# camillabelponer/dealii-slod

Measured on NVIDIA B200. Metric: slod_basis_patches_per_s, higher is better.
Workload: dtype f64

## Files before the change

### dealii-slod_b200/csrc/kernels.cu

```cuda
#include <cuda_runtime.h>
#include <math.h>
#include <stdint.h>
#include <stdio.h>
#include <stdlib.h>

#include "geom.h"
#include "kernels.h"

namespace slod {

__constant__ Params cP;

cudaError_t upload_params(const Params &p, cudaStream_t st) {
  return cudaMemcpyToSymbolAsync(cP, &p, sizeof(Params), 0, cudaMemcpyHostToDevice, st);
}

__device__ __forceinline__ int nfields() { return cP.problem == 0 ? 1 : 2; }

__device__ void load_coef(const Geom &g, const double *__restrict__ d_coef, double *sCoef, int t0 = -1, int nt = 0) {
  if (t0 < 0) { t0 = threadIdx.x; nt = blockDim.x; }
  const int n = cP.n;
  const int msx = g.m[0] * n, msy = g.m[1] * n, msz = (cP.dim == 3) ? g.m[2] * n : 1;
  const int nsubp = msx * msy * msz;
  const long long nsub = cP.nsub;
// ... 790 lines not shown
        x0[j] = max(gq.lo[0] * n, ulo[0]);
        x1[j] = min((gq.lo[0] + gq.m[0]) * n, uhi[0]);
        if (x1[j] < x0[j]) continue;
        qid[j] = (int)morton_fast(qc, DIM);
        lox[j] = gq.lo[0] * n;
        px[j] = gq.p[0];
        ux0 = min(ux0, x0[j]);
        ux1 = max(ux1, x1[j]);
        if (!got) {
          got = true;
          b0y = max(gq.lo[1] * n, ulo[1]);
          b1y = min((gq.lo[1] + gq.m[1]) * n, uhi[1]);
          loy = gq.lo[1] * n;
          py = gq.p[1];
          if (DIM == 3) {
            b0z = max(gq.lo[2] * n, ulo[2]);
            b1z = min((gq.lo[2] + gq.m[2]) * n, uhi[2]);
            loz = gq.lo[2] * n;
          } else {
            b0z = 0; b1z = 0; loz = 0;
          }
        }
      }
      if (!got || b1y < b0y || b1z < b0z) continue;
      const int exu = ux1 - ux0 + 1, ey = b1y - b0y + 1, ez = b1z - b0z + 1;
      for (int e = 0; e < S; ++e) {
        double acc[NQ][NA];
#pragma unroll
        for (int j = 0; j < NQ; ++j)
#pragma unroll
          for (int k = 0; k < NA; ++k) acc[j][k] = 0.0;
        for (int t = lane; t < exu * ey; t += 32) {
          const int iy = t / exu, ix = t - iy * exu;
          const int gx = ux0 + ix, gy = b0y + iy;
          const double *u1 = sU + (((b0z - ulo[2]) * NU + (gy - ulo[1])) * NU + (gx - ulo[0])) * S;
          const double *q1[NQ];
          int sq[NQ];
          bool in[NQ];
#pragma unroll
          for (int j = 0; j < NQ; ++j) {
            in[j] = gx >= x0[j] && gx <= x1[j];
            sq[j] = px[j] * py * S;
            q1[j] = aphi + ((size_t)qid[j] * S + e) * lay.nf_max +
                    (((b0z - loz) * py + (gy - loy)) * px[j] + (in[j] ? gx - lox[j] : 0)) * S;
          }
          for (int iz = 0; iz < ez; ++iz) {
#pragma unroll
            for (int c = 0; c < S; ++c) {
              double v[NQ];
#pragma unroll
              for (int j = 0; j < NQ; ++j) v[j] = in[j] ? q1[j][iz * sq[j] + c] : 0.0;
              const double *u = u1 + iz * NU * NU * S + c;
#pragma unroll
              for (int k = 0; k < NA; ++k) {
                const double uk = u[(size_t)k * NUV * S];
#pragma unroll
                for (int j = 0; j < NQ; ++j) acc[j][k] += v[j] * uk;
              }
            }
          }
        }
#pragma unroll
        for (int j = 0; j < NQ; ++j) {
          if (x1[j] < x0[j]) continue;
          const double val = warp_sum_packed(acc[j], lane);
          if ((lane & (NA == 8 ? 3 : 7)) == 0) {
            const int k = warp_sum_index<NA>(lane);
            const int mem = k / S, d = k - mem * S;
            if (sGeo[mem][7]) {
              const int Dx = qx0 + j - sGeo[mem][3], Dy = qy - sGeo[mem][4], Dz = (DIM == 3) ? qz - sGeo[mem][5] : 0;
              if (abs(Dx) <= w && abs(Dy) <= w && abs(Dz) <= w) {
                const int slot = (DIM == 3) ? ((Dz + w) * ww + (Dy + w)) * ww + (Dx + w) : (Dy + w) * ww + (Dx + w);
                Kell[((size_t)sGeo[mem][6] * S + d) * cP.ell_width + slot * S + e] = val;
              }
            }
          }
        }
      }
    }
  }
}
template <int DIM, int S>
static cudaError_t launch_coarse_blocked_t(int grid, size_t smem, cudaStream_t st, int p0, int p1, const double *phi,
                                           const double *aphi, double *Kell, const FinishLayout &lay, int NU,
                                           const int *groups, int n_groups) {
  if (groups) {
    cudaError_t e = cudaFuncSetAttribute(k_coarse_blocked<DIM, S, true>, cudaFuncAttributeMaxDynamicSharedMemorySize, (int)smem);
    if (e != cudaSuccess) return e;
    k_coarse_blocked<DIM, S, true><<<grid, kCoarseThreads, smem, st>>>(p0, p1, groups, n_groups, phi, aphi, Kell, lay, NU);
    return cudaGetLastError();
  }
  cudaError_t e = cudaFuncSetAttribute(k_coarse_blocked<DIM, S, false>, cudaFuncAttributeMaxDynamicSharedMemorySize, (int)smem);
  if (e != cudaSuccess) return e;
  e = cudaMemsetAsync(Kell + (size_t)p0 * S * (lay.ell_width), 0, sizeof(double) * (size_t)(p1 - p0) * S * lay.ell_width, st);
  if (e != cudaSuccess) return e;
  k_coarse_blocked<DIM, S, false><<<grid, kCoarseThreads, smem, st>>>(p0, p1, nullptr, 0, phi, aphi, Kell, lay, NU);
  return cudaGetLastError();
}
size_t coarse_blocked_smem(int dim, int s, int NU) {
  size_t nuv = (dim == 3) ? (size_t)NU * NU * NU : (size_t)NU * NU;
  return sizeof(double) * ((size_t)(1 << dim) * s * nuv * s);
}
cudaError_t launch_coarse_blocked(int dim, int s, int grid, size_t smem, cudaStream_t st, int p0, int p1,
                                  const double *phi, const double *aphi, double *Kell, const FinishLayout &lay, int NU,
                                  const int *groups, int n_groups) {
  if (dim == 3 && s == 1) return launch_coarse_blocked_t<3, 1>(grid, smem, st, p0, p1, phi, aphi, Kell, lay, NU, groups, n_groups);
  if (dim == 2 && s == 1) return launch_coarse_blocked_t<2, 1>(grid, smem, st, p0, p1, phi, aphi, Kell, lay, NU, groups, n_groups);
  if (dim == 2 && s == 2) return launch_coarse_blocked_t<2, 2>(grid, smem, st, p0, p1, phi, aphi, Kell, lay, NU, groups, n_groups);
  return cudaErrorInvalidValue;
}

cudaError_t launch_patch_solve(int grid, size_t smem, cudaStream_t st, const int *ids, int n_work, const double *coef,
                               double *X, double *Lws, int *status, const SolveLayout &lay) {
  cudaError_t e = cudaFuncSetAttribute(k_patch_solve<kSolveNB>, cudaFuncAttributeMaxDynamicSharedMemorySize, (int)smem);
  if (e != cudaSuccess) return e;
  k_patch_solve<kSolveNB><<<grid, lay.threads, smem, st>>>(ids, n_work, coef, X, Lws, status, lay);
  return cudaGetLastError();
}
template <int RBMAX, int NW>
static cudaError_t launch_mma_t(int grid, size_t smem, cudaStream_t st, const int *ids, int n_work, const double *coef,
                                double *X, double *Lws, int *status, const SolveMmaLayout &lay, int *work_counter) {
  cudaError_t e = cudaFuncSetAttribute(k_patch_solve_mma<RBMAX, NW>, cudaFuncAttributeMaxDynamicSharedMemorySize, (int)smem);
  if (e != cudaSuccess) return e;
  k_patch_solve_mma<RBMAX, NW><<<grid, 32 * NW, smem, st>>>(ids, n_work, coef, X, Lws, status, lay, work_counter);
  return cudaGetLastError();
}
size_t solve_mma_smem(int variant, int coef_doubles, int nip_max, int stw) {
  const int RBMAX = (variant == 0) ? 13 : 4;
  const int NW = (variant == 0) ? 16 : (variant == 1 ? 4 : 8);
  const int R = 8 * RBMAX, LDWF = (R % 16 == 8) ? R : R + 8, LDP = R + 4;
  return sizeof(double) * ((size_t)coef_doubles + (size_t)R * LDWF + 8 * LDP + kSolveStages * (R * 8 + 64) +
                           (size_t)nip_max * stw) +
         sizeof(int) * ((size_t)nip_max + 8 * NW + RBMAX * (RBMAX - 1) / 2 + 32 + 8);
}
cudaError_t launch_patch_solve_mma(int variant, int grid, size_t smem, cudaStream_t st, const int *ids, int n_work,
                                   const double *coef, double *X, double *Lws, int *status, int coef_doubles, int ldx,
                                   long long x_stride, long long lws_per_cta, int nip_max, int stw, int *work_counter) {
  SolveMmaLayout lay{coef_doubles, nip_max, stw, ldx, x_stride, lws_per_cta};
  if (work_counter) {
    cudaError_t e = cudaMemsetAsync(work_counter, 0, sizeof(int), st);
    if (e != cudaSuccess) return e;
  }
  switch (variant) {
    case 0: return launch_mma_t<13, 16>(grid, smem, st, ids, n_work, coef, X, Lws, status, lay, work_counter);
    case 1: return launch_mma_t<4, 4>(grid, smem, st, ids, n_work, coef, X, Lws, status, lay, work_counter);
    case 2: return launch_mma_t<4, 8>(grid, smem, st, ids, n_work, coef, X, Lws, status, lay, work_counter);
  }
  return cudaErrorInvalidValue;
}

constexpr int kSplitRB = 13, kFactorWarps = 8, kTriWarps = 16;
size_t split_factor_smem(int coef_doubles, int nip_max) {
  const int R = 8 * kSplitRB, LDWF = (R % 16 == 8) ? R : R + 8, LDP = R + 4;
  return sizeof(double) * ((size_t)coef_doubles + (size_t)R * LDWF + 8 * LDP + 2 * 64 + 64) +
         sizeof(int) * ((size_t)nip_max + kSplitRB * (kSplitRB - 1) / 2 + 16 + 8);
}
size_t split_trisolve_smem(int nip_max) {
  return sizeof(double) * ((size_t)kTriStages * kSplitRB * 64) + 2 * kTriStages * sizeof(unsigned long long) +
         sizeof(int) * ((size_t)nip_max + 8 * kTriWarps + kTriWarps + nip_max / 8 + 1 + 8 + 4);
}
long long split_rec_stride(int nip_max) { return (long long)(nip_max / 8) * kSplitRB * 64; }
size_t split_stencil_ws_doubles(int grid, int nip_max) { return (size_t)grid * nip_max * 14; }
cudaError_t launch_patch_factor(int grid, size_t smem, cudaStream_t st, const int *ids, int n_work, const double *coef,
                                double *Lrec, double *stencil_ws, int *status, int coef_doubles, int nip_max, int ldx,
                                long long x_stride, int *work_counter) {
  SplitLayout lay{coef_doubles, nip_max, ldx, x_stride, split_rec_stride(nip_max)};
  cudaError_t e = cudaFuncSetAttribute(k_patch_factor<kSplitRB, kFactorWarps>, cudaFuncAttributeMaxDynamicSharedMemorySize, (int)smem);
  if (e != cudaSuccess) return e;
  e = cudaFuncSetAttribute(k_patch_factor<kSplitRB, kFactorWarps>, cudaFuncAttributePreferredSharedMemoryCarveout,
                           (int)cudaSharedmemCarveoutMaxShared);
  if (e != cudaSuccess) return e;
  if (getenv("SLOD_PRINT_OCC")) {
    int nb = 0;
    cudaOccupancyMaxActiveBlocksPerMultiprocessor(&nb, k_patch_factor<kSplitRB, kFactorWarps>, 32 * kFactorWarps, smem);
    printf("k_patch_factor: %d CTAs/SM, %zu B dynamic shared memory\n", nb, smem);
  }
  if (work_counter && (e = cudaMemsetAsync(work_counter, 0, sizeof(int), st)) != cudaSuccess) return e;
  k_patch_factor<kSplitRB, kFactorWarps><<<grid, 32 * kFactorWarps, smem, st>>>(ids, n_work, coef, Lrec, stencil_ws, status, lay, work_counter);
  return cudaGetLastError();
}
cudaError_t launch_patch_trisolve(int grid, size_t smem, cudaStream_t st, const int *ids, int n_work, const double *Lrec,
                                  double *X, int coef_doubles, int nip_max, int ldx, long long x_stride, int *work_counter) {
  SplitLayout lay{coef_doubles, nip_max, ldx, x_stride, split_rec_stride(nip_max)};
  cudaError_t e = cudaFuncSetAttribute(k_patch_trisolve<kSplitRB, kTriWarps>, cudaFuncAttributeMaxDynamicSharedMemorySize, (int)smem);
  if (e != cudaSuccess) return e;
  if (work_counter && (e = cudaMemsetAsync(work_counter, 0, sizeof(int), st)) != cudaSuccess) return e;
  k_patch_trisolve<kSplitRB, kTriWarps><<<grid, 32 * kTriWarps, smem, st>>>(ids, n_work, Lrec, X, lay, work_counter);
  return cudaGetLastError();
}

cudaError_t launch_patch_dense(int grid, size_t smem, cudaStream_t st, const int *ids, int n_work, const double *coef,
                               const double *X, double *Minv, double *G, double *diag, int *status,
                               const DenseLayout &lay) {
  cudaError_t e = cudaFuncSetAttribute(k_patch_dense, cudaFuncAttributeMaxDynamicSharedMemorySize, (int)smem);
  if (e != cudaSuccess) return e;
  k_patch_dense<<<grid, lay.threads, smem, st>>>(ids, n_work, coef, X, Minv, G, diag, status, lay);
  return cudaGetLastError();
}
template <int NTILE>
static cudaError_t launch_dense_t(int grid, size_t smem, cudaStream_t st, const int *ids, int n_work, const double *coef,
                                  const double *X, const double *W, double *Minv, double *G, double *diag, int *status,
                                  const DenseLayout &lay, int *work_counter) {
  cudaError_t e = cudaFuncSetAttribute(k_patch_dense_mma<NTILE>, cudaFuncAttributeMaxDynamicSharedMemorySize, (int)smem);
  if (e != cudaSuccess) return e;
  k_patch_dense_mma<NTILE><<<grid, 32 * NTILE, smem, st>>>(ids, n_work, coef, X, W, Minv, G, diag, status, lay, work_counter);
  return cudaGetLastError();
}
size_t dense_mma_smem(int ntile, int coef_doubles, int nb_max) {
  (void)nb_max;
  (void)coef_doubles;
  const int NC = 8 * ntile, LDM = NC + 4;
  return sizeof(double) * ((size_t)NC * LDM + 2 * (size_t)kDTB * LDM) + sizeof(int) * ((size_t)NC * 32 + 8);
}
cudaError_t launch_patch_dense_mma(int ntile, int grid, size_t smem, cudaStream_t st, const int *ids, int n_work,
                                   const double *coef, const double *X, const double *W, double *Minv, double *G,
                                   double *diag, int *status, const DenseLayout &lay, int *work_counter) {
  if (work_counter) {
    cudaError_t e = cudaMemsetAsync(work_counter, 0, sizeof(int), st);
    if (e != cudaSuccess) return e;
  }
  switch (ntile) {
    case 4: return launch_dense_t<4>(grid, smem, st, ids, n_work, coef, X, W, Minv, G, diag, status, lay, work_counter);
    case 8: return launch_dense_t<8>(grid, smem, st, ids, n_work, coef, X, W, Minv, G, diag, status, lay, work_counter);
    case 16: return launch_dense_t<16>(grid, smem, st, ids, n_work, coef, X, W, Minv, G, diag, status, lay, work_counter);
  }
  return cudaErrorInvalidValue;
}
size_t flux_smem(int coef_doubles, int ldx, int nb_max) {
  (void)ldx;
  return sizeof(double) * ((size_t)coef_doubles + (size_t)kFTB * kFNB) +
         sizeof(int) * ((size_t)kFTB * kFNB + kFTB + nb_max + 8);
}
cudaError_t launch_patch_flux(int grid, size_t smem, cudaStream_t st, const int *ids, int n_work, const double *coef,
                              const double *X, double *W, const FluxLayout &lay, int *work_counter) {
  cudaError_t e = cudaFuncSetAttribute(k_patch_flux, cudaFuncAttributeMaxDynamicSharedMemorySize, (int)smem);
  if (e != cudaSuccess) return e;
  if (work_counter && (e = cudaMemsetAsync(work_counter, 0, sizeof(int), st)) != cudaSuccess) return e;
  k_patch_flux<<<grid, 256, smem, st>>>(ids, n_work, coef, X, W, lay, work_counter);
  return cudaGetLastError();
}

size_t select_fast_smem(int ncd_max) {
  const size_t nbk = (size_t)(ncd_max + 6) / 8;
  return sizeof(double) * (nbk * (nbk + 1) / 2 * 64 + 8 * nbk + 8);
}
size_t select_jacobi_smem(int ncd_max) {
  return sizeof(double) * ((size_t)ncd_max * (ncd_max + 1) / 2 + (size_t)ncd_max * ncd_max + 6 * (size_t)ncd_max) +
         sizeof(int) * (3 * (size_t)ncd_max + 8);
}
size_t eig_tridiag_smem(int nmax) { return sizeof(double) * ((size_t)nmax * (nmax | 1) + 4 * (size_t)nmax); }
size_t eig_ql_smem(int nmax) { return sizeof(double) * 8 * 3 * (size_t)nmax; }
size_t eig_finish_smem(int nmax) {
  return sizeof(double) * ((size_t)nmax * kEigLd + 5 * (size_t)nmax) + sizeof(int) * ((size_t)nmax + 8);
}

cudaError_t launch_select_pipeline(const SelectPlan &pl, cudaStream_t st, const int *ids, int n_work, const double *Minv,
                                   const double *G, double *cvec, double *diag, int *status, const SelectBuffers &b,
                                   int *n_launches) {
  cudaError_t e;
#define SLOD_ATTR(k, sm)                                                                        \
  if ((e = cudaFuncSetAttribute(k, cudaFuncAttributeMaxDynamicSharedMemorySize, (int)(sm))) != cudaSuccess) return e
  SLOD_ATTR(k_select_fast, pl.smem_fast);
  SLOD_ATTR(k_select_jacobi, pl.smem_jac);
  if ((e = cudaMemsetAsync(b.counters, 0, 4 * sizeof(int), st)) != cudaSuccess) return e;
  k_select_fast<<<min(n_work, pl.grid_fast), 256, pl.smem_fast, st>>>(
      ids, n_work, Minv, G, cvec, diag, b.counters, pl.use_ql ? b.eig_list : b.jac_list, pl.use_ql ? 1 : 2, pl.lay);
  ++*n_launches;
  if (pl.use_ql) {
    SLOD_ATTR(k_eig_tridiag<4>, pl.smem_tri);
    SLOD_ATTR(k_eig_tridiag<8>, pl.smem_tri);
    SLOD_ATTR(k_eig_ql, pl.smem_ql);
    SLOD_ATTR(k_eig_finish, pl.smem_fin);
    const long long items_max = (long long)n_work * pl.s;
    for (long long off = 0; off < items_max; off += pl.eig.cap_items) {
      if (pl.eig.nmax - 1 <= 128)
        k_eig_tridiag<4><<<pl.grid_tri, 512, pl.smem_tri, st>>>(ids, b.counters, b.eig_list, (int)off, G, b.H, b.V, pl.eig);
      else
        k_eig_tridiag<8><<<pl.grid_tri, 512, pl.smem_tri, st>>>(ids, b.counters, b.eig_list, (int)off, G, b.H, b.V, pl.eig);
      k_eig_ql<<<pl.grid_ql, 256, pl.smem_ql, st>>>(ids, b.counters, b.eig_list, (int)off, b.V, b.rot_cs, b.rot_i,
                                                   b.rot_n, pl.eig);
      k_eig_finish<<<pl.grid_fin, 128, pl.smem_fin, st>>>(ids, b.counters, b.eig_list, (int)off, Minv, b.H, b.V,
                                                         b.rot_cs, b.rot_i, b.rot_n, cvec, diag, b.jac_list, pl.eig);
      *n_launches += 3;
    }
  }
  k_select_jacobi<<<pl.grid_jac, pl.lay.threads, pl.smem_jac, st>>>(ids, b.counters, b.jac_list, Minv, G, cvec, diag,
                                                                    status, pl.lay);
  ++*n_launches;
#undef SLOD_ATTR
  return cudaGetLastError();
}
cudaError_t launch_patch_finish(int grid, size_t smem, cudaStream_t st, const int *ids, int n_work, const double *coef,
                                const double *X, const double *cvec, double *phi, double *aphi,
                                const FinishLayout &lay) {
  cudaError_t e = cudaFuncSetAttribute(k_patch_finish, cudaFuncAttributeMaxDynamicSharedMemorySize, (int)smem);
  if (e != cudaSuccess) return e;
  k_patch_finish<<<grid, 256, smem, st>>>(ids, n_work, coef, X, cvec, phi, aphi, lay);
  return cudaGetLastError();
}
__global__ void __launch_bounds__(256)
k_gather(const double *__restrict__ src, const long long *__restrict__ perm, double *__restrict__ dst, long long n) {
  for (long long i = blockIdx.x * (long long)blockDim.x + threadIdx.x; i < n; i += (long long)gridDim.x * blockDim.x)
    dst[i] = src[perm[i]];
}
cudaError_t launch_gather(cudaStream_t st, const double *src, const long long *perm, double *dst, long long n) {
  if (n <= 0) return cudaSuccess;
  k_gather<<<148 * 8, 256, 0, st>>>(src, perm, dst, n);
  return cudaGetLastError();
// ... 245 lines not shown
```

### dealii-slod_b200/csrc/solve_split.cuh

```cuda
#pragma once
#include <cuda/std/cstdint>

namespace slod {

__device__ __forceinline__ uint32_t smem_u32(const void *p) { return (uint32_t)__cvta_generic_to_shared(p); }
__device__ __forceinline__ void mbar_init(uint64_t *bar, int count) {
  asm volatile("mbarrier.init.shared::cta.b64 [%0], %1;" ::"r"(smem_u32(bar)), "r"(count) : "memory");
}
__device__ __forceinline__ void mbar_expect_tx(uint64_t *bar, uint32_t bytes) {
  asm volatile("mbarrier.arrive.expect_tx.shared::cta.b64 _, [%0], %1;" ::"r"(smem_u32(bar)), "r"(bytes) : "memory");
}
__device__ __forceinline__ void mbar_arrive(uint64_t *bar) {
  asm volatile("mbarrier.arrive.shared::cta.b64 _, [%0];" ::"r"(smem_u32(bar)) : "memory");
}
__device__ __forceinline__ void mbar_arrive_n(uint64_t *bar, int count) {
  asm volatile("mbarrier.arrive.shared::cta.b64 _, [%0], %1;" ::"r"(smem_u32(bar)), "r"(count) : "memory");
}
__device__ __forceinline__ bool mbar_try_wait(uint64_t *bar, uint32_t parity) {
  uint32_t ok;
  asm volatile(
      "{\n\t.reg .pred p;\n\tmbarrier.try_wait.parity.shared::cta.b64 p, [%1], %2;\n\tselp.u32 %0, 1, 0, p;\n\t}"
      : "=r"(ok)
      : "r"(smem_u32(bar)), "r"(parity)
      : "memory");
  return ok != 0;
}
__device__ __forceinline__ void mbar_wait(uint64_t *bar, uint32_t parity) {
  while (!mbar_try_wait(bar, parity)) {
  }
}
__device__ __forceinline__ void bulk_g2s(void *dst, const void *src, uint32_t bytes, uint64_t *bar) {
  asm volatile("cp.async.bulk.shared::cluster.global.mbarrier::complete_tx::bytes [%0], [%1], %2, [%3];" ::"r"(
                   smem_u32(dst)),
               "l"(src), "r"(bytes), "r"(smem_u32(bar))
               : "memory");
}

__device__ __forceinline__ void dmma1688(double &c0, double &c1, double &c2, double &c3, double a0, double a1, double a2,
                                         double a3, double b0, double b1) {
  asm volatile(
      "mma.sync.aligned.m16n8k8.row.col.f64.f64.f64.f64 {%0,%1,%2,%3}, {%4,%5,%6,%7}, {%8,%9}, {%0,%1,%2,%3};\n"
      : "+d"(c0), "+d"(c1), "+d"(c2), "+d"(c3)
      : "d"(a0), "d"(a1), "d"(a2), "d"(a3), "d"(b0), "d"(b1));
}

#ifdef SLOD_PHASE_CLOCKS
#define PHS_DECL(wa, wb, wc) long long ph_acc[12] = {0}; long long ph_last = clock64(); const bool ph_on = (blockIdx.x == 0) && ((threadIdx.x & 31) == 0) && ((threadIdx.x >> 5) == (wa) || (threadIdx.x >> 5) == (wb) || (threadIdx.x >> 5) == (wc));
#else
#define PHS_DECL(wa, wb, wc)
#endif

constexpr int kTriStages = 12;

struct SplitLayout {
  int coef_doubles;
  int nip_max;
  int ldx;
  long long x_stride;
  long long rec_stride;
};

__device__ __forceinline__ int frag_pos(int r, int c) { return 8 * r + 2 * (c & 3) + (c >> 2); }

__device__ __forceinline__ double stiff_entry_3d(const Geom &g, const double *sCoef, const double *sK, int n,
                                                 const int a[3], const int dl[3]) {
  const int msx = g.m[0] * n, msy = g.m[1] * n;
  double acc = 0.0;
#pragma unroll
  for (int oc = 0; oc < 8; ++oc) {
    const int bx = oc & 1, by = (oc >> 1) & 1, bz = (oc >> 2) & 1;
    const bool ok = (dl[0] == 0 || dl[0] == (bx ? 1 : -1)) && (dl[1] == 0 || dl[1] == (by ? 1 : -1)) &&
                    (dl[2] == 0 || dl[2] == (bz ? 1 : -1));
    const int ox = a[0] - 1 + bx, oy = a[1] - 1 + by, oz = a[2] - 1 + bz;
    const int la = (1 - bx) + 2 * (1 - by) + 4 * (1 - bz);
    const int lb = (1 - bx + dl[0]) + 2 * (1 - by + dl[1]) + 4 * (1 - bz + dl[2]);
    const double c = sCoef[(oz * msy + oy) * msx + ox];
    const double kv = sK[(la * 8 + lb) & 63];
    acc += ok ? c * kv : 0.0;
  }
  return acc;
}

template <int RBMAX, int NW>
__global__ void __launch_bounds__(32 * NW, 2)
k_patch_factor(const int *__restrict__ patch_ids, int n_work, const double *__restrict__ d_coef,
               double *__restrict__ Lrec, double *__restrict__ stencil_ws, int *__restrict__ status, SplitLayout lay,
               int *work_counter) {
  constexpr int R = 8 * RBMAX;
  constexpr int LDWF = (R % 16 == 8) ? R : R + 8;
  constexpr int LDP = R + 4;
  constexpr int NT = 32 * NW;
  constexpr int LSTEP = RBMAX * 64;
  constexpr int NTT = RBMAX * (RBMAX - 1) / 2;
  extern __shared__ double smem[];
  double *sCoef = smem;
  double *sWf = sCoef + lay.coef_doubles;
  double *sLpT = sWf + R * LDWF;
  double *sLinv = sLpT + 8 * LDP;
  double *sK = sLinv + 2 * 64;
  int *sRowPk = (int *)(sK + 64);
  int *sTileTab = sRowPk + lay.nip_max;
  int *sDOff = sTileTab + NTT;
  const int tid = threadIdx.x, lane = tid & 31, warp = tid >> 5;
  const int g = lane >> 2, t = lane & 3;
  constexpr int nlow = 13;

  for (int tt = tid; tt < NTT; tt += NT) {
    int offI = 1;
    while ((offI + 1) * offI / 2 <= tt) ++offI;
    sTileTab[tt] = offI | ((tt - offI * (offI - 1) / 2 + 1) << 8);
  }
  for (int i = tid; i < 64; i += NT) sK[i] = cP.Kref[i];

  unsigned long long table_key = ~0ull;
  __shared__ int sNextWork;
  SLOD_WORK_LOOP(w, n_work, work_counter, sNextWork) {
    fetch_work_item(w, work_counter, &sNextWork);
    const int pid = patch_ids[w];
    const Geom geo = make_geom(cP, pid);
    const int Ni = geo.Ni, bw = geo.bw, n = cP.n;
    const bool rebuild = (shape_key(geo) != table_key);
    table_key = shape_key(geo);
    const int NBLK = (Ni + 7) >> 3;
    int RB = (bw + 8 + 7) >> 3;
    if (RB > RBMAX) RB = RBMAX;
    double *rec = Lrec + (size_t)w * lay.rec_stride;
    double *stw = stencil_ws + (size_t)blockIdx.x * lay.nip_max * (nlow + 1);
    __syncthreads();
    load_coef(geo, d_coef, sCoef);
    if (rebuild)
    for (int r = tid; r < 8 * NBLK; r += NT) {
      int pk = 0;
      if (r < Ni) {
        int a[3];
        interior_coords(geo, r, a);
        int mask = 0;
        for (int e = 0; e <= nlow; ++e) {
          int dl[3];
          lower_offset(e, dl);
          bool inside = true;
#pragma unroll
          for (int x = 0; x < 3; ++x) inside = inside && (a[x] + dl[x] >= 1 && a[x] + dl[x] <= geo.p[x] - 2);
          if (inside) mask |= 1 << e;
        }
        pk = a[0] | (a[1] << 5) | (a[2] << 10) | (mask << 16) | (1 << 31);
      }
      sRowPk[r] = pk;
    }
    if (tid <= nlow) {
      int dl[3];
      lower_offset(tid, dl);
      sDOff[tid] = dl[0] + geo.q[0] * (dl[1] + geo.q[1] * dl[2]);
    }
    __syncthreads();

    auto zero_block_row = [&](int sB) {
      for (int item = tid; item < 32 * RB; item += NT) {
        const int i = item & 7, q = item >> 3;
        *reinterpret_cast<double2 *>(sWf + (8 * sB + i) * LDWF + 2 * q) = make_double2(0.0, 0.0);
      }
    };
    auto stencil_item = [&](int blk, int item) -> double {
      const int i = item & 7, e = item >> 3;
      const int pk = sRowPk[8 * blk + i];
      if (pk >= 0) return (e == 0) ? 1.0 : 0.0;
      if (!((pk >> (16 + e)) & 1)) return 0.0;
      const int a[3] = {pk & 31, (pk >> 5) & 31, (pk >> 10) & 31};
      int dl[3];
      lower_offset(e, dl);
      return stiff_entry_3d(geo, sCoef, sK, n, a, dl);
    };
    auto scatter_item = [&](int blk, int sB, int item, double v) {
      const int i = item & 7, e = item >> 3;
      const int r = 8 * blk + i;
      const int pk = sRowPk[r];
      if (pk < 0) {
        if (!((pk >> (16 + e)) & 1)) return;
        const int c = r + sDOff[e];
        int sb = sB - (blk - (c >> 3));
        if (sb < 0) sb += RB;
        sWf[(8 * sB + i) * LDWF + 8 * sb + (c & 7)] = v;
      } else if (e == 0) {
        sWf[(8 * sB + i) * LDWF + 8 * sB + i] = 1.0;
      }
    };

    for (int b = 0; b < RB && b < NBLK; ++b) zero_block_row(b);
    for (int item = tid; item < NBLK * 8 * (nlow + 1); item += NT)
      __stcg(stw + item, stencil_item(item / (8 * (nlow + 1)), item % (8 * (nlow + 1))));
    __syncthreads();
    for (int b = 0; b < RB && b < NBLK; ++b) {
      for (int item = tid; item < 8 * (nlow + 1); item += NT) {
        const double v = __ldcg(stw + b * 8 * (nlow + 1) + item);
        scatter_item(b, b, item, v);
      }
    }
    __syncthreads();
    int bad = 0;
    if (warp == 0) bad |= chol8_inv_reg(sWf, LDWF, lane, sLinv);
    __syncthreads();

    PHS_DECL(0, 3, 4)
    constexpr int NTW = NW - NW / 4;
    constexpr int NBAR = 32 * (NTW + 1);
    constexpr int NBAR2 = 32 * (NTW + 2);
    constexpr bool kW4Tiles = (RBMAX == 13 && NTW == 6);
    constexpr int NIT = (8 * (nlow + 1) + 31) / 32;
    double vnext[NIT];
#pragma unroll
    for (int j = 0; j < NIT; ++j)
      vnext[j] = (warp == 4 && RB < NBLK && lane + 32 * j < 8 * (nlow + 1)) ? __ldcg(stw + RB * 8 * (nlow + 1) + lane + 32 * j) : 0.0;
    for (int k = 0, kslot = 0; k < NBLK; ++k, kslot = (kslot + 1 == RB) ? 0 : kslot + 1) {
      PH(0)
      const int cur = k & 1;
      const double *Linv = sLinv + cur * 64;
      int nl = NBLK - 1 - k;
      if (nl > RB - 1) nl = RB - 1;
      double *Ls = rec + (size_t)k * LSTEP;
      const int ntile = nl * (nl + 1) / 2;
      const double binv0 = Linv[g * 8 + t], binv1 = Linv[g * 8 + 4 + t];
      auto panel_tile = [&](int off) {
        int sI = kslot + off;
        if (sI >= RB) sI -= RB;
        const double *wt = sWf + (8 * sI + g) * LDWF + 8 * kslot;
        double p0 = 0.0, p1 = 0.0;
        dmma884(p0, p1, wt[t], binv0);
        dmma884(p0, p1, wt[4 + t], binv1);
        sLpT[(2 * t) * LDP + 8 * sI + g] = p0;
        sLpT[(2 * t + 1) * LDP + 8 * sI + g] = p1;
        double *dst = Ls + 64 * off;
        dst[frag_pos(g, 2 * t)] = p0;
        dst[frag_pos(g, 2 * t + 1)] = p1;
      };
      auto sweep_row = [&](int offI, int jlo, int jhi) {
        if (offI > nl) return;
        int sI = kslot + offI;
        if (sI >= RB) sI -= RB;
        const double a0 = -sLpT[t * LDP + 8 * sI + g], a1 = -sLpT[(4 + t) * LDP + 8 * sI + g];
        double *rowp = sWf + (8 * sI + g) * LDWF + 2 * t;
        for (int offJ = jlo; offJ <= jhi; offJ += 3) {
          double2 c[3];
          double b0[3], b1[3];
          int sJ[3];
#pragma unroll
          for (int u = 0; u < 3; ++u) {
            const int oj = (offJ + u <= jhi) ? offJ + u : offJ;
            sJ[u] = kslot + oj;
            if (sJ[u] >= RB) sJ[u] -= RB;
            c[u] = *reinterpret_cast<double2 *>(rowp + 8 * sJ[u]);
            b0[u] = sLpT[t * LDP + 8 * sJ[u] + g];
            b1[u] = sLpT[(4 + t) * LDP + 8 * sJ[u] + g];
          }
#pragma unroll
          for (int u = 0; u < 3; ++u) dmma884(c[u].x, c[u].y, a0, b0[u]);
#pragma unroll
          for (int u = 0; u < 3; ++u) dmma884(c[u].x, c[u].y, a1, b1[u]);
#pragma unroll
          for (int u = 0; u < 3; ++u)
            if (offJ + u <= jhi) *reinterpret_cast<double2 *>(rowp + 8 * sJ[u]) = c[u];
        }
      };
      if (warp == 0) {
        if (nl >= 1) {
          panel_tile(1);
          __syncwarp();
          asm volatile("bar.arrive 1, %0;" ::"n"(NBAR) : "memory");
          if (kW4Tiles) asm volatile("bar.arrive 2, %0;" ::"n"(NBAR2) : "memory");
          int sI = kslot + 1;
          if (sI >= RB) sI -= RB;
          double *ct = sWf + (8 * sI + g) * LDWF + 8 * sI + 2 * t;
          double2 c = *reinterpret_cast<double2 *>(ct);
          const double a0 = -sLpT[t * LDP + 8 * sI + g], a1 = -sLpT[(4 + t) * LDP + 8 * sI + g];
          dmma884(c.x, c.y, a0, -a0);
          dmma884(c.x, c.y, a1, -a1);
          *reinterpret_cast<double2 *>(ct) = c;
          __syncwarp();
          PH(6)
          bad |= chol8_inv_reg(sWf + (8 * sI) * LDWF + 8 * sI, LDWF, lane, sLinv + (cur ^ 1) * 64);
          PH(7)
        }
      } else if ((warp & 3) == 0) {
        if (warp == 4) {
          *reinterpret_cast<double2 *>(Ls + 2 * lane) = make_double2(Linv[g * 8 + t], Linv[g * 8 + 4 + t]);
          if (k + RB < NBLK) {
            double v[NIT];
#pragma unroll
            for (int j = 0; j < NIT; ++j) {
              v[j] = vnext[j];
              vnext[j] = (k + RB + 1 < NBLK && lane + 32 * j < 8 * (nlow + 1))
                             ? __ldcg(stw + (k + RB + 1) * 8 * (nlow + 1) + lane + 32 * j) : 0.0;
            }
            for (int item = lane; item < 32 * RB; item += 32) {
              const int i = item & 7, q = item >> 3;
              *reinterpret_cast<double2 *>(sWf + (8 * kslot + i) * LDWF + 2 * q) = make_double2(0.0, 0.0);
            }
            __syncwarp();
#pragma unroll
            for (int j = 0; j < NIT; ++j)
              if (lane + 32 * j < 8 * (nlow + 1)) scatter_item(k + RB, kslot, lane + 32 * j, v[j]);
          }
          PH(8)
          if (RBMAX == 13 && NTW == 6) {
            if (nl >= 1) asm volatile("bar.sync 2, %0;" ::"n"(NBAR2) : "memory");
            PH(9)
#pragma unroll 1
            for (int r0 = RBMAX - 1; r0 >= RBMAX - 6; r0 -= 3) {
              double *ct[3];
              double2 c[3];
              double a0[3], a1[3];
#pragma unroll
              for (int u = 0; u < 3; ++u) {
                int sI = kslot + (r0 - u);
                if (sI >= RB) sI -= RB;
                ct[u] = sWf + (8 * sI + g) * LDWF + 8 * sI + 2 * t;
                c[u] = *reinterpret_cast<double2 *>(ct[u]);
                a0[u] = -sLpT[t * LDP + 8 * sI + g];
                a1[u] = -sLpT[(4 + t) * LDP + 8 * sI + g];
              }
#pragma unroll
              for (int u = 0; u < 3; ++u) dmma884(c[u].x, c[u].y, a0[u], -a0[u]);
#pragma unroll
              for (int u = 0; u < 3; ++u) dmma884(c[u].x, c[u].y, a1[u], -a1[u]);
#pragma unroll
              for (int u = 0; u < 3; ++u)
                if (r0 - u <= nl) *reinterpret_cast<double2 *>(ct[u]) = c[u];
            }
          }
        }
      } else {
        const int wrank = warp - 1 - (warp >> 2);
        for (int off = 2 + wrank; off <= nl; off += NTW) panel_tile(off);
        PH(1)
        if (nl >= 1 && kW4Tiles) {
          __syncwarp();
          asm volatile("bar.arrive 2, %0;" ::"n"(NBAR2) : "memory");
        }
        if (nl >= 1) asm volatile("bar.sync 1, %0;" ::"n"(NBAR) : "memory");
        PH(3)
        if (RBMAX == 13 && NTW == 6) {
          sweep_row(1 + wrank, (wrank == 0) ? 2 : 1, 1 + wrank);
          sweep_row(RBMAX - 1 - wrank, 1, RBMAX - 2 - wrank);
        } else
        for (int tt = 1 + wrank; tt < ntile; tt += 3 * NTW) {
          double *ct[3];
          double2 c[3];
          double a0[3], a1[3], b0[3], b1[3];
#pragma unroll
          for (int u = 0; u < 3; ++u) {
            const int tu = tt + u * NTW;
            const int tab = sTileTab[tu < ntile ? tu : tt];
            const int offI = tab & 0xff, offJ = tab >> 8;
            int sI = kslot + offI, sJ = kslot + offJ;
            if (sI >= RB) sI -= RB;
            if (sJ >= RB) sJ -= RB;
            ct[u] = sWf + (8 * sI + g) * LDWF + 8 * sJ + 2 * t;
            c[u] = *reinterpret_cast<double2 *>(ct[u]);
            a0[u] = -sLpT[t * LDP + 8 * sI + g];
            a1[u] = -sLpT[(4 + t) * LDP + 8 * sI + g];
            b0[u] = sLpT[t * LDP + 8 * sJ + g];
            b1[u] = sLpT[(4 + t) * LDP + 8 * sJ + g];
          }
#pragma unroll
          for (int u = 0; u < 3; ++u) dmma884(c[u].x, c[u].y, a0[u], b0[u]);
#pragma unroll
          for (int u = 0; u < 3; ++u) dmma884(c[u].x, c[u].y, a1[u], b1[u]);
#pragma unroll
          for (int u = 0; u < 3; ++u)
            if (tt + u * NTW < ntile) *reinterpret_cast<double2 *>(ct[u]) = c[u];
        }
      }
      PH(4)
      __syncthreads();
      PH(5)
    }
    PH_PRINT("factor")
    if (bad && lane == 0) atomicOr(&status[pid], 1);
  }
}

template <int RBMAX, int NW>
__global__ void __launch_bounds__(32 * NW, 1)
k_patch_trisolve(const int *__restrict__ patch_ids, int n_work, const double *__restrict__ Lrec,
                 double *__restrict__ Xbuf, SplitLayout lay, int *work_counter) {
  constexpr int NT = 32 * NW;
  constexpr int NC = 8 * NW;
  constexpr int LSTEP = RBMAX * 64;
  constexpr int NSTG = kTriStages;
  extern __shared__ __align__(128) double smem[];
  double *sRing = smem;
  uint64_t *sFull = reinterpret_cast<uint64_t *>(sRing + NSTG * LSTEP);
  uint64_t *sEmpty = sFull + NSTG;
  int *sRowPk = reinterpret_cast<int *>(sEmpty + NSTG);
  int *sColCell = sRowPk + lay.nip_max;
  int *sKstart = sColCell + NC;
  int *sNskip = sKstart + NW;
  volatile uint32_t *sProgress = reinterpret_cast<volatile uint32_t *>(sNskip + lay.nip_max / 8 + 1);
  const int tid = threadIdx.x, lane = tid & 31, warp = tid >> 5;
  const int g = lane >> 2, t = lane & 3;
  const int tpos = 8 * t + 2 * (g & 3) + (g >> 2);
  const int grp = (NW == 16) ? (warp < 8 ? ((0x86543210u >> (4 * warp)) & 15) : ((0xCFED9BA7u >> (4 * (warp - 8))) & 15))
                             : warp;
  const bool is_prod = (grp == NW - 1) && (lane == 0);

  if (tid == 0) {
    for (int s = 0; s < NSTG; ++s) {
      mbar_init(sFull + s, 1);
      mbar_init(sEmpty + s, NW);
    }
    asm volatile("fence.mbarrier_init.release.cluster;" ::: "memory");
    asm volatile("fence.proxy.async.shared::cta;" ::: "memory");
    *sProgress = 0;
  }
  __syncthreads();
  uint32_t rec_base = 0;
  unsigned long long table_key = ~0ull;

  __shared__ int sNextWork;
  SLOD_WORK_LOOP(w, n_work, work_counter, sNextWork) {
    fetch_work_item(w, work_counter, &sNextWork);
    const int pid = patch_ids[w];
    const Geom geo = make_geom(cP, pid);
    const int Ni = geo.Ni, bw = geo.bw, ncd = geo.Ncd;
    const int NBLK = (Ni + 7) >> 3;
    int RB = (bw + 8 + 7) >> 3;
    if (RB > RBMAX) RB = RBMAX;
    double *X = Xbuf + (size_t)w * lay.x_stride;
    const double *rec = Lrec + (size_t)w * lay.rec_stride;
    const bool rebuild = (shape_key(geo) != table_key);
    table_key = shape_key(geo);
    __syncthreads();
    if (rebuild)
    for (int r = tid; r < 8 * NBLK; r += NT) {
      int pk = 0;
      if (r < Ni) {
        int a[3];
        interior_coords(geo, r, a);
        pk = a[0] | (a[1] << 5) | (a[2] << 10) | (1 << 31);
      }
      sRowPk[r] = pk;
    }
    if (rebuild)
    for (int col = tid; col < NC; col += NT) {
      int v = -1;
      if (col < ncd) {
        int kc[3];
        zcol_to_cell(geo, col, kc);
        v = kc[0] | (kc[1] << 5) | (kc[2] << 10);
      }
      sColCell[col] = v;
    }
    __syncthreads();
    const int mycc0 = sColCell[8 * grp + 2 * t], mycc1 = sColCell[8 * grp + 2 * t + 1];
    const int n = cP.n;
    int kstart, kend;
    {
      int first = 1 << 30, last = -1;
      const int cc = sColCell[8 * grp + (lane & 7)];
      if (cc >= 0) {
        const int kz = (cc >> 10) & 31;
        int plo = n * kz, phi_ = n * kz + n;
        if (plo < 1) plo = 1;
        if (phi_ > geo.p[2] - 2) phi_ = geo.p[2] - 2;
        first = (plo - 1) * geo.q[0] * geo.q[1];
        last = phi_ * geo.q[0] * geo.q[1] - 1;
      }
#pragma unroll
      for (int o = 4; o > 0; o >>= 1) {
        first = min(first, __shfl_xor_sync(0xffffffffu, first, o));
        last = max(last, __shfl_xor_sync(0xffffffffu, last, o));
      }
      kstart = (last < 0) ? NBLK : first >> 3;
      kend = last >> 3;
      if (lane == 0) sKstart[warp] = kstart;
    }
    __syncthreads();
    if (rebuild)
    for (int k = tid; k <= NBLK; k += NT) {
      int cnt = 0;
      for (int w2 = 0; w2 < NW; ++w2) cnt += (k < NBLK) ? (sKstart[w2] > k) : (sKstart[w2] >= NBLK);
      sNskip[k] = cnt;
    }
    __syncthreads();
    const int pw_hi = __double2hiint(cP.pw), pw_lo = __double2loint(cP.pw);
    auto rhs_tile = [&](int blk, double &c0, double &c1) {
      if (blk < kstart || blk > kend) {
        c0 = c1 = 0.0;
        return;
      }
      const int pk = sRowPk[8 * blk + g];
      int hi[2];
#pragma unroll
      for (int h = 0; h < 2; ++h) {
        const int cc = h ? mycc1 : mycc0;
        bool in = (pk < 0) && (cc >= 0);
        int cnt = 0;
#pragma unroll
        for (int x = 0; x < 3; ++x) {
          const int tt = ((pk >> (5 * x)) & 31) - n * ((cc >> (5 * x)) & 31);
          in = in && (tt >= 0) && (tt <= n);
          cnt += (tt != 0 && tt != n) ? 1 : 0;
        }
        hi[h] = in ? pw_hi + (cnt << 20) : 0;
      }
      c0 = __hiloint2double(hi[0], hi[0] ? pw_lo : 0);
      c1 = __hiloint2double(hi[1], hi[1] ? pw_lo : 0);
    };

    const int total = 2 * NBLK;
    int issued = 0;
    auto step_of = [&](int i) { return i < NBLK ? i : 2 * NBLK - 1 - i; };
    auto top_up = [&](int upto) {
      if (upto > total) upto = total;
      while (issued < upto) {
        const uint32_t r = rec_base + issued;
        const int slot = r % NSTG;
        const uint32_t use = r / NSTG;
        if (use > 0) mbar_wait(sEmpty + slot, (use - 1) & 1);
        const int k = step_of(issued);
        int nl = NBLK - 1 - k;
        if (nl > RB - 1) nl = RB - 1;
        const uint32_t bytes = 8u * 64u * (1 + nl);
        mbar_expect_tx(sFull + slot, bytes);
        bulk_g2s(sRing + slot * LSTEP, rec + (size_t)k * LSTEP, bytes, sFull + slot);
        const int nskip = sNskip[issued < NBLK ? k : NBLK];
        if (nskip > 0) mbar_arrive_n(sEmpty + slot, nskip);
// ... 149 lines not shown
```

Baseline: 221,400.

## Replace per-step block barrier in patch factor with double-buffered named barriers

Replaces the per-iteration __syncthreads in the blocked Cholesky factor loop with parity-alternating named barriers, and double-buffers the panel (sLpT) so the next step's panel can be written while the current one is still read. Warp 0 can start the next diagonal block as soon as the row-2 sweep finishes, instead of waiting for all warps. The initial stencil scatter goes straight into the window without a round trip through global memory, and the generic tile-table path is dropped. The kernel is now hardwired to RB=13 and 8 warps, and the finer barrier protocol carries a risk of races or deadlock.

```diff
diff --git a/dealii-slod_b200/csrc/kernels.cu b/dealii-slod_b200/csrc/kernels.cu
--- a/dealii-slod_b200/csrc/kernels.cu
+++ b/dealii-slod_b200/csrc/kernels.cu
@@ -966,8 +966,8 @@
 constexpr int kSplitRB = 13, kFactorWarps = 8, kTriWarps = 16;
 size_t split_factor_smem(int coef_doubles, int nip_max) {
   const int R = 8 * kSplitRB, LDWF = (R % 16 == 8) ? R : R + 8, LDP = R + 4;
-  return sizeof(double) * ((size_t)coef_doubles + (size_t)R * LDWF + 8 * LDP + 2 * 64 + 64) +
-         sizeof(int) * ((size_t)nip_max + kSplitRB * (kSplitRB - 1) / 2 + 16 + 8);
+  return sizeof(double) * ((size_t)coef_doubles + (size_t)R * LDWF + 2 * 8 * LDP + 2 * 64 + 64) +
+         sizeof(int) * ((size_t)nip_max + 16 + 8);
 }
 size_t split_trisolve_smem(int nip_max) {
   return sizeof(double) * ((size_t)kTriStages * kSplitRB * 64) + 2 * kTriStages * sizeof(unsigned long long) +
diff --git a/dealii-slod_b200/csrc/solve_split.cuh b/dealii-slod_b200/csrc/solve_split.cuh
--- a/dealii-slod_b200/csrc/solve_split.cuh
+++ b/dealii-slod_b200/csrc/solve_split.cuh
@@ -81,41 +81,52 @@
   return acc;
 }
 
+template <int ID, int NTHREADS>
+__device__ __forceinline__ void nbar_sync(int parity) {
+  if (parity) asm volatile("bar.sync %0, %1;" ::"n"(ID + 1), "n"(NTHREADS) : "memory");
+  else asm volatile("bar.sync %0, %1;" ::"n"(ID), "n"(NTHREADS) : "memory");
+}
+template <int ID, int NTHREADS>
+__device__ __forceinline__ void nbar_arrive(int parity) {
+  if (parity) asm volatile("bar.arrive %0, %1;" ::"n"(ID + 1), "n"(NTHREADS) : "memory");
+  else asm volatile("bar.arrive %0, %1;" ::"n"(ID), "n"(NTHREADS) : "memory");
+}
+constexpr int kBarLinv = 1;
+constexpr int kBarPanel = 3;
+constexpr int kBarPanel4 = 5;
+constexpr int kBarRow2 = 7;
+constexpr int kBarStep = 9;
+
 template <int RBMAX, int NW>
 __global__ void __launch_bounds__(32 * NW, 2)
 k_patch_factor(const int *__restrict__ patch_ids, int n_work, const double *__restrict__ d_coef,
                double *__restrict__ Lrec, double *__restrict__ stencil_ws, int *__restrict__ status, SplitLayout lay,
                int *work_counter) {
+  static_assert(RBMAX == 13 && NW == 8, "the role split assumes 13 window blocks and 8 warps");
   constexpr int R = 8 * RBMAX;
   constexpr int LDWF = (R % 16 == 8) ? R : R + 8;
   constexpr int LDP = R + 4;
   constexpr int NT = 32 * NW;
   constexpr int LSTEP = RBMAX * 64;
-  constexpr int NTT = RBMAX * (RBMAX - 1) / 2;
   extern __shared__ double smem[];
   double *sCoef = smem;
   double *sWf = sCoef + lay.coef_doubles;
   double *sLpT = sWf + R * LDWF;
-  double *sLinv = sLpT + 8 * LDP;
+  double *sLinv = sLpT + 2 * 8 * LDP;
   double *sK = sLinv + 2 * 64;
   int *sRowPk = (int *)(sK + 64);
-  int *sTileTab = sRowPk + lay.nip_max;
-  int *sDOff = sTileTab + NTT;
+  int *sDOff = sRowPk + lay.nip_max;
   const int tid = threadIdx.x, lane = tid & 31, warp = tid >> 5;
   const int g = lane >> 2, t = lane & 3;
   constexpr int nlow = 13;
 
-  for (int tt = tid; tt < NTT; tt += NT) {
-    int offI = 1;
-    while ((offI + 1) * offI / 2 <= tt) ++offI;
-    sTileTab[tt] = offI | ((tt - offI * (offI - 1) / 2 + 1) << 8);
-  }
   for (int i = tid; i < 64; i += NT) sK[i] = cP.Kref[i];
 
   unsigned long long table_key = ~0ull;
   __shared__ int sNextWork;
   SLOD_WORK_LOOP(w, n_work, work_counter, sNextWork) {
     fetch_work_item(w, work_counter, &sNextWork);
+    PHS_DECL(0, 3, 4)
     const int pid = patch_ids[w];
     const Geom geo = make_geom(cP, pid);
     const int Ni = geo.Ni, bw = geo.bw, n = cP.n;
@@ -152,7 +163,6 @@
       lower_offset(tid, dl);
       sDOff[tid] = dl[0] + geo.q[0] * (dl[1] + geo.q[1] * dl[2]);
     }
-    __syncthreads();
 
     auto zero_block_row = [&](int sB) {
       for (int item = tid; item < 32 * RB; item += NT) {
@@ -186,26 +196,26 @@
     };
 
     for (int b = 0; b < RB && b < NBLK; ++b) zero_block_row(b);
-    for (int item = tid; item < NBLK * 8 * (nlow + 1); item += NT)
-      __stcg(stw + item, stencil_item(item / (8 * (nlow + 1)), item % (8 * (nlow + 1))));
-    __syncthreads();
-    for (int b = 0; b < RB && b < NBLK; ++b) {
-      for (int item = tid; item < 8 * (nlow + 1); item += NT) {
-        const double v = __ldcg(stw + b * 8 * (nlow + 1) + item);
-        scatter_item(b, b, item, v);
-      }
+    __syncthreads();
+    for (int item = tid; item < NBLK * 8 * (nlow + 1); item += NT) {
+      const int b = item / (8 * (nlow + 1)), e = item % (8 * (nlow + 1));
+      const double v = stencil_item(b, e);
+      if (b < RB) scatter_item(b, b, e, v);
+      else __stcg(stw + item, v);
     }
     __syncthreads();
     int bad = 0;
     if (warp == 0) bad |= chol8_inv_reg(sWf, LDWF, lane, sLinv);
     __syncthreads();
-
-    PHS_DECL(0, 3, 4)
+    PH(10)
+
     constexpr int NTW = NW - NW / 4;
-    constexpr int NBAR = 32 * (NTW + 1);
-    constexpr int NBAR2 = 32 * (NTW + 2);
-    constexpr bool kW4Tiles = (RBMAX == 13 && NTW == 6);
+    constexpr int NPAN = 32 * (NTW + 1);
+    constexpr int NPAN4 = 32 * (NTW + 2);
+    constexpr int NSTEP = 32 * (NTW + 1);
     constexpr int NIT = (8 * (nlow + 1) + 31) / 32;
+    const int wrank = warp - 1 - (warp >> 2);
+    const bool full_sync = (RB <= 2);
     double vnext[NIT];
 #pragma unroll
     for (int j = 0; j < NIT; ++j)
@@ -214,10 +224,15 @@
       PH(0)
       const int cur = k & 1;
       const double *Linv = sLinv + cur * 64;
+      double *Lp = sLpT + cur * 8 * LDP;
       int nl = NBLK - 1 - k;
       if (nl > RB - 1) nl = RB - 1;
       double *Ls = rec + (size_t)k * LSTEP;
-      const int ntile = nl * (nl + 1) / 2;
+      if (k > 0) {
+        if (warp == 0) nbar_sync<kBarRow2, 64>(cur ^ 1);
+        else nbar_sync<kBarLinv, NT>(cur ^ 1);
+      }
+      PH(1)
       const double binv0 = Linv[g * 8 + t], binv1 = Linv[g * 8 + 4 + t];
       auto panel_tile = [&](int off) {
         int sI = kslot + off;
@@ -226,8 +241,8 @@
         double p0 = 0.0, p1 = 0.0;
         dmma884(p0, p1, wt[t], binv0);
         dmma884(p0, p1, wt[4 + t], binv1);
-        sLpT[(2 * t) * LDP + 8 * sI + g] = p0;
-        sLpT[(2 * t + 1) * LDP + 8 * sI + g] = p1;
+        Lp[(2 * t) * LDP + 8 * sI + g] = p0;
+        Lp[(2 * t + 1) * LDP + 8 * sI + g] = p1;
         double *dst = Ls + 64 * off;
         dst[frag_pos(g, 2 * t)] = p0;
         dst[frag_pos(g, 2 * t + 1)] = p1;
@@ -236,7 +251,7 @@
         if (offI > nl) return;
         int sI = kslot + offI;
         if (sI >= RB) sI -= RB;
-        const double a0 = -sLpT[t * LDP + 8 * sI + g], a1 = -sLpT[(4 + t) * LDP + 8 * sI + g];
+        const double a0 = -Lp[t * LDP + 8 * sI + g], a1 = -Lp[(4 + t) * LDP + 8 * sI + g];
         double *rowp = sWf + (8 * sI + g) * LDWF + 2 * t;
         for (int offJ = jlo; offJ <= jhi; offJ += 3) {
           double2 c[3];
@@ -248,8 +263,8 @@
             sJ[u] = kslot + oj;
             if (sJ[u] >= RB) sJ[u] -= RB;
             c[u] = *reinterpret_cast<double2 *>(rowp + 8 * sJ[u]);
-            b0[u] = sLpT[t * LDP + 8 * sJ[u] + g];
-            b1[u] = sLpT[(4 + t) * LDP + 8 * sJ[u] + g];
+            b0[u] = Lp[t * LDP + 8 * sJ[u] + g];
+            b1[u] = Lp[(4 + t) * LDP + 8 * sJ[u] + g];
           }
 #pragma unroll
           for (int u = 0; u < 3; ++u) dmma884(c[u].x, c[u].y, a0, b0[u]);
@@ -261,116 +276,90 @@
         }
       };
       if (warp == 0) {
+        *reinterpret_cast<double2 *>(Ls + 2 * lane) = make_double2(binv0, binv1);
         if (nl >= 1) {
           panel_tile(1);
           __syncwarp();
-          asm volatile("bar.arrive 1, %0;" ::"n"(NBAR) : "memory");
-          if (kW4Tiles) asm volatile("bar.arrive 2, %0;" ::"n"(NBAR2) : "memory");
+          nbar_arrive<kBarPanel, NPAN>(cur);
+          nbar_arrive<kBarPanel4, NPAN4>(cur);
           int sI = kslot + 1;
           if (sI >= RB) sI -= RB;
           double *ct = sWf + (8 * sI + g) * LDWF + 8 * sI + 2 * t;
           double2 c = *reinterpret_cast<double2 *>(ct);
-          const double a0 = -sLpT[t * LDP + 8 * sI + g], a1 = -sLpT[(4 + t) * LDP + 8 * sI + g];
+          const double a0 = -Lp[t * LDP + 8 * sI + g], a1 = -Lp[(4 + t) * LDP + 8 * sI + g];
           dmma884(c.x, c.y, a0, -a0);
           dmma884(c.x, c.y, a1, -a1);
           *reinterpret_cast<double2 *>(ct) = c;
           __syncwarp();
           PH(6)
           bad |= chol8_inv_reg(sWf + (8 * sI) * LDWF + 8 * sI, LDWF, lane, sLinv + (cur ^ 1) * 64);
+          nbar_arrive<kBarLinv, NT>(cur);
           PH(7)
         }
-      } else if ((warp & 3) == 0) {
-        if (warp == 4) {
-          *reinterpret_cast<double2 *>(Ls + 2 * lane) = make_double2(Linv[g * 8 + t], Linv[g * 8 + 4 + t]);
-          if (k + RB < NBLK) {
-            double v[NIT];
-#pragma unroll
-            for (int j = 0; j < NIT; ++j) {
-              v[j] = vnext[j];
-              vnext[j] = (k + RB + 1 < NBLK && lane + 32 * j < 8 * (nlow + 1))
-                             ? __ldcg(stw + (k + RB + 1) * 8 * (nlow + 1) + lane + 32 * j) : 0.0;
-            }
-            for (int item = lane; item < 32 * RB; item += 32) {
-              const int i = item & 7, q = item >> 3;
-              *reinterpret_cast<double2 *>(sWf + (8 * kslot + i) * LDWF + 2 * q) = make_double2(0.0, 0.0);
-            }
-            __syncwarp();
-#pragma unroll
-            for (int j = 0; j < NIT; ++j)
-              if (lane + 32 * j < 8 * (nlow + 1)) scatter_item(k + RB, kslot, lane + 32 * j, v[j]);
+      } else if (warp == 4) {
+        if (k + RB < NBLK) {
+          double v[NIT];
+#pragma unroll
+          for (int j = 0; j < NIT; ++j) {
+            v[j] = vnext[j];
+            vnext[j] = (k + RB + 1 < NBLK && lane + 32 * j < 8 * (nlow + 1))
+                           ? __ldcg(stw + (k + RB + 1) * 8 * (nlow + 1) + lane + 32 * j) : 0.0;
           }
-          PH(8)
-          if (RBMAX == 13 && NTW == 6) {
-            if (nl >= 1) asm volatile("bar.sync 2, %0;" ::"n"(NBAR2) : "memory");
-            PH(9)
+          for (int item = lane; item < 32 * RB; item += 32) {
+            const int i = item & 7, q = item >> 3;
+            *reinterpret_cast<double2 *>(sWf + (8 * kslot + i) * LDWF + 2 * q) = make_double2(0.0, 0.0);
+          }
+          __syncwarp();
+#pragma unroll
+          for (int j = 0; j < NIT; ++j)
+            if (lane + 32 * j < 8 * (nlow + 1)) scatter_item(k + RB, kslot, lane + 32 * j, v[j]);
+        }
+        PH(8)
+        if (nl >= 1) nbar_sync<kBarPanel4, NPAN4>(cur);
+        PH(3)
 #pragma unroll 1
-            for (int r0 = RBMAX - 1; r0 >= RBMAX - 6; r0 -= 3) {
-              double *ct[3];
-              double2 c[3];
-              double a0[3], a1[3];
-#pragma unroll
-              for (int u = 0; u < 3; ++u) {
-                int sI = kslot + (r0 - u);
-                if (sI >= RB) sI -= RB;
-                ct[u] = sWf + (8 * sI + g) * LDWF + 8 * sI + 2 * t;
-                c[u] = *reinterpret_cast<double2 *>(ct[u]);
-                a0[u] = -sLpT[t * LDP + 8 * sI + g];
-                a1[u] = -sLpT[(4 + t) * LDP + 8 * sI + g];
-              }
-#pragma unroll
-              for (int u = 0; u < 3; ++u) dmma884(c[u].x, c[u].y, a0[u], -a0[u]);
-#pragma unroll
-              for (int u = 0; u < 3; ++u) dmma884(c[u].x, c[u].y, a1[u], -a1[u]);
-#pragma unroll
-              for (int u = 0; u < 3; ++u)
-                if (r0 - u <= nl) *reinterpret_cast<double2 *>(ct[u]) = c[u];
-            }
-          }
-        }
-      } else {
-        const int wrank = warp - 1 - (warp >> 2);
-        for (int off = 2 + wrank; off <= nl; off += NTW) panel_tile(off);
-        PH(1)
-        if (nl >= 1 && kW4Tiles) {
-          __syncwarp();
-          asm volatile("bar.arrive 2, %0;" ::"n"(NBAR2) : "memory");
-        }
-        if (nl >= 1) asm volatile("bar.sync 1, %0;" ::"n"(NBAR) : "memory");
-        PH(3)
-        if (RBMAX == 13 && NTW == 6) {
-          sweep_row(1 + wrank, (wrank == 0) ? 2 : 1, 1 + wrank);
-          sweep_row(RBMAX - 1 - wrank, 1, RBMAX - 2 - wrank);
-        } else
-        for (int tt = 1 + wrank; tt < ntile; tt += 3 * NTW) {
+        for (int r0 = RBMAX - 1; r0 >= RBMAX - 6; r0 -= 3) {
           double *ct[3];
           double2 c[3];
-          double a0[3], a1[3], b0[3], b1[3];
+          double a0[3], a1[3];
 #pragma unroll
           for (int u = 0; u < 3; ++u) {
-            const int tu = tt + u * NTW;
-            const int tab = sTileTab[tu < ntile ? tu : tt];
-            const int offI = tab & 0xff, offJ = tab >> 8;
-            int sI = kslot + offI, sJ = kslot + offJ;
+            int sI = kslot + (r0 - u);
             if (sI >= RB) sI -= RB;
-            if (sJ >= RB) sJ -= RB;
-            ct[u] = sWf + (8 * sI + g) * LDWF + 8 * sJ + 2 * t;
+            ct[u] = sWf + (8 * sI + g) * LDWF + 8 * sI + 2 * t;
             c[u] = *reinterpret_cast<double2 *>(ct[u]);
-            a0[u] = -sLpT[t * LDP + 8 * sI + g];
-            a1[u] = -sLpT[(4 + t) * LDP + 8 * sI + g];
-            b0[u] = sLpT[t * LDP + 8 * sJ + g];
-            b1[u] = sLpT[(4 + t) * LDP + 8 * sJ + g];
+            a0[u] = -Lp[t * LDP + 8 * sI + g];
+            a1[u] = -Lp[(4 + t) * LDP + 8 * sI + g];
           }
 #pragma unroll
-          for (int u = 0; u < 3; ++u) dmma884(c[u].x, c[u].y, a0[u], b0[u]);
-#pragma unroll
-          for (int u = 0; u < 3; ++u) dmma884(c[u].x, c[u].y, a1[u], b1[u]);
+          for (int u = 0; u < 3; ++u) dmma884(c[u].x, c[u].y, a0[u], -a0[u]);
+#pragma unroll
+          for (int u = 0; u < 3; ++u) dmma884(c[u].x, c[u].y, a1[u], -a1[u]);
 #pragma unroll
           for (int u = 0; u < 3; ++u)
-            if (tt + u * NTW < ntile) *reinterpret_cast<double2 *>(ct[u]) = c[u];
-        }
-      }
-      PH(4)
-      __syncthreads();
+            if (r0 - u <= nl) *reinterpret_cast<double2 *>(ct[u]) = c[u];
+        }
+        PH(4)
+        nbar_sync<kBarStep, NSTEP>(0);
+      } else {
+        for (int off = 2 + wrank; off <= nl; off += NTW) panel_tile(off);
+        PH(2)
+        if (nl >= 1) {
+          __syncwarp();
+          nbar_arrive<kBarPanel4, NPAN4>(cur);
+          nbar_sync<kBarPanel, NPAN>(cur);
+        }
+        PH(3)
+        sweep_row(1 + wrank, (wrank == 0) ? 2 : 1, 1 + wrank);
+        if (wrank == 1 && nl >= 1) {
+          __syncwarp();
+          nbar_arrive<kBarRow2, 64>(cur);
+        }
+        sweep_row(RBMAX - 1 - wrank, 1, RBMAX - 2 - wrank);
+        PH(4)
+        nbar_sync<kBarStep, NSTEP>(0);
+      }
+      if (full_sync) __syncthreads();
       PH(5)
     }
     PH_PRINT("factor")
```

New measurement: 220,300, median of 6. No clear change (-0.5%).
